# MuMuJun97/semantic_slam_mapping

Hardware: AMD Instinct MI355X
Metric: frames/sec semantic-mapping, 640x480 RGB-D (higher is better)
Workload: dtype u8; 1 GPU; configs[1]: synthetic 640x480 RGB-D + precomputed 12-class masks, 1k frames per GPU, ORB 1000 kp/frame, 5 ref frames, leaf 0.10 m; frames_per_gpu=1000, frames_all_gpus=1000, batch_frames=250, matcher_halo_frames=0, parallelism=single GPU

## Files before the change

### semantic_slam_mapping_amd/csrc/kernels_map.hip

```cpp
#include "ssm_internal.h"
#include <cstring>
#include <cmath>

#define MK_W 64
#define MK_H 16
__global__ void __launch_bounds__(256)
mask_kernel(const uint8_t* __restrict__ sem, int w, int h, int tiles_x, uint8_t* __restrict__ mask)
{
    __shared__ uint8_t m0[MK_H + 4][MK_W + 4];
    __shared__ uint8_t m1[MK_H + 4][MK_W];
    const int tx0 = (blockIdx.x % tiles_x) * MK_W, ty0 = (blockIdx.x / tiles_x) * MK_H;
    const uint8_t* s = sem + (size_t)blockIdx.y * w * h * 3;
    for (int i = threadIdx.x; i < (MK_H + 4) * (MK_W + 4); i += 256) {
        const int ly = i / (MK_W + 4), lx = i - ly * (MK_W + 4);
        const int gx = tx0 + lx - 2, gy = ty0 + ly - 2;
        uint8_t v = 0;
        if (gx >= 0 && gx < w && gy >= 0 && gy < h) {
            const uint8_t* p = s + ((size_t)gy * w + gx) * 3;
            const int b = p[0], g = p[1], r = p[2];
            v = ((b == 0 && g == 64 && r == 64) || (b == 192 && g == 128 && r == 0)) ? 255 : 0;
        }
        m0[ly][lx] = v;
    }
    __syncthreads();
    for (int i = threadIdx.x; i < (MK_H + 4) * MK_W; i += 256) {
        const int ly = i / MK_W, lx = i - ly * MK_W;
        const uint8_t* p = &m0[ly][lx];
        m1[ly][lx] = p[0] | p[1] | p[2] | p[3] | p[4];
    }
    __syncthreads();
    uint8_t* dst = mask + (size_t)blockIdx.y * w * h;
    const int lx = threadIdx.x & 63;
    for (int ly = threadIdx.x >> 6; ly < MK_H; ly += 4) {
        const int gx = tx0 + lx, gy = ty0 + ly;
        if (gx < w && gy < h) dst[(size_t)gy * w + gx] = m1[ly][lx] | m1[ly+1][lx] | m1[ly+2][lx] | m1[ly+3][lx] | m1[ly+4][lx];
    }
}
hipError_t k_moving_mask(const uint8_t* sem, int n, int w, int h, uint8_t* mask, hipStream_t s)
{
    const int tx = (w + MK_W - 1) / MK_W, ty = (h + MK_H - 1) / MK_H;
    mask_kernel<<<dim3(tx * ty, n), 256, 0, s>>>(sem, w, h, tx, mask);
    return hipGetLastError();
}

#define BP_PIX 1024
int backproject_chunks(int w, int h) { return (w * h + BP_PIX - 1) / BP_PIX; }

__device__ __forceinline__ bool bp_keep(int d, int mk, int b, int g, int r, double maxd)
{
    if (d == 0) return false;
    if ((double)d > maxd) return false;
    if (mk == 255) return false;
    if ((b == 128 && g == 128 && r == 128) || (b == 128 && g == 192 && r == 192) || (b == 192 && g == 128 && r == 0)) return false;
    return true;
}
__global__ void __launch_bounds__(256)
bp_count_kernel(const uint16_t* __restrict__ depth, const uint8_t* __restrict__ sem, const uint8_t* __restrict__ mask,
                int npix, double maxd, int chunks, int32_t* __restrict__ chunk_cnt)
{
    __shared__ int wsum[4];
    const size_t fo = (size_t)blockIdx.y * npix;
    const int p0 = blockIdx.x * BP_PIX + threadIdx.x * 4;
    int c = 0;
#pragma unroll
    for (int i = 0; i < 4; i++) {
        const int p = p0 + i;
        if (p < npix) {
            const uint8_t* s = sem + (fo + p) * 3;
            c += bp_keep(depth[fo + p], mask[fo + p], s[0], s[1], s[2], maxd);
        }
    }
#pragma unroll
    for (int o = 32; o > 0; o >>= 1) c += __shfl_xor(c, o, 64);
    if ((threadIdx.x & 63) == 0) wsum[threadIdx.x >> 6] = c;
    __syncthreads();
    if (threadIdx.x == 0) chunk_cnt[blockIdx.y * chunks + blockIdx.x] = wsum[0] + wsum[1] + wsum[2] + wsum[3];
}
__global__ void __launch_bounds__(1024)
bp_scan_kernel(const int32_t* __restrict__ chunk_cnt, int n, int chunks, int64_t* __restrict__ chunk_off,
               int32_t* __restrict__ npoints, int64_t* __restrict__ total)
{
    __shared__ long long part[1024];
    const int tot = n * chunks, tid = threadIdx.x;
    const int per = (tot + 1023) / 1024;
    const int b = tid * per, e = min(b + per, tot);
    long long s = 0;
    for (int i = b; i < e; i++) s += chunk_cnt[i];
    part[tid] = s;
    __syncthreads();
    for (int o = 1; o < 1024; o <<= 1) {
        long long v = tid >= o ? part[tid - o] : 0;
        __syncthreads();
        part[tid] += v;
        __syncthreads();
    }
    long long run = part[tid] - s;
    for (int i = b; i < e; i++) { chunk_off[i] = run; run += chunk_cnt[i]; }
    if (tid == 1023) *total = part[1023];
    __syncthreads();
    for (int f = tid; f < n; f += 1024) {
        int t = 0;
        for (int c = 0; c < chunks; c++) t += chunk_cnt[f * chunks + c];
        npoints[f] = t;
    }
}
__global__ void __launch_bounds__(256)
bp_emit_kernel(const uint16_t* __restrict__ depth, const uint8_t* __restrict__ rgb, const uint8_t* __restrict__ sem,
               const uint8_t* __restrict__ mask, const double* __restrict__ pose, int w, int npix, ssm_camera cam, double maxd,
               int chunks, const int64_t* __restrict__ chunk_off, ssm_point* __restrict__ out)
{
    __shared__ int wsum[4];
    const size_t fo = (size_t)blockIdx.y * npix;
    const int p0 = blockIdx.x * BP_PIX + threadIdx.x * 4;
    const int lane = threadIdx.x & 63, wv = threadIdx.x >> 6;
    bool k[4]; int c = 0;
#pragma unroll
    for (int i = 0; i < 4; i++) {
        const int p = p0 + i; k[i] = false;
        if (p < npix) {
            const uint8_t* s = sem + (fo + p) * 3;
            k[i] = bp_keep(depth[fo + p], mask[fo + p], s[0], s[1], s[2], maxd);
        }
        c += k[i];
    }
    int inc = c;
#pragma unroll
    for (int o = 1; o < 64; o <<= 1) { const int v = __shfl_up(inc, o, 64); if (lane >= o) inc += v; }
    if (lane == 63) wsum[wv] = inc;
    __syncthreads();
    int off = inc - c;
    for (int i = 0; i < wv; i++) off += wsum[i];
    if (c == 0) return;
    ssm_point* dst = out + chunk_off[blockIdx.y * chunks + blockIdx.x] + off;
    double T[12];
    const bool hasT = pose != nullptr;
    if (hasT) { const double* P = pose + (size_t)blockIdx.y * 16;
#pragma unroll
        for (int j = 0; j < 4; j++) { T[3*j] = P[4*j]; T[3*j+1] = P[4*j+1]; T[3*j+2] = P[4*j+2]; } }
#pragma unroll
    for (int i = 0; i < 4; i++) {
        if (!k[i]) continue;
        const int p = p0 + i;
        const int v = p / w, u = p - v * w;
        const int d = depth[fo + p];
        const float z = (float)((double)d / cam.scale);
        const float x = (float)(((double)u - cam.cx) * (double)z / cam.fx);
        const float y = (float)(((double)v - cam.cy) * (double)z / cam.fy);
        float ox = x, oy = y, oz = z;
        if (hasT) {
            const double X = x, Y = y, Z = z;
            ox = (float)(T[0] * X + T[3] * Y + T[6] * Z + T[9]);
            oy = (float)(T[1] * X + T[4] * Y + T[7] * Z + T[10]);
            oz = (float)(T[2] * X + T[5] * Y + T[8] * Z + T[11]);
        }
        const uint8_t* c3 = rgb + (fo + p) * 3;
        const uint8_t* s3 = sem + (fo + p) * 3;
        const int sb = s3[0], sg = s3[1], sr = s3[2];
        uint32_t label = 255;
        switch ((sb << 16) | (sg << 8) | sr) {
            case (128 << 16) | (128 << 8) | 128: label = 0; break;   case (0 << 16) | (0 << 8) | 128: label = 1; break;
            case (128 << 16) | (192 << 8) | 192: label = 2; break;   case (0 << 16) | (69 << 8) | 255: label = 3; break;
            case (128 << 16) | (64 << 8) | 128: label = 4; break;    case (222 << 16) | (40 << 8) | 60: label = 5; break;
            case (0 << 16) | (128 << 8) | 128: label = 6; break;     case (128 << 16) | (128 << 8) | 192: label = 7; break;
            case (128 << 16) | (64 << 8) | 64: label = 8; break;     case (128 << 16) | (0 << 8) | 64: label = 9; break;
            case (0 << 16) | (64 << 8) | 64: label = 10; break;      case (192 << 16) | (128 << 8) | 0: label = 11; break;
        }
        uint4 lo, hi;
        lo.x = __float_as_uint(ox); lo.y = __float_as_uint(oy); lo.z = __float_as_uint(oz); lo.w = __float_as_uint(1.0f);
        hi.x = (uint32_t)c3[0] | ((uint32_t)c3[1] << 8) | ((uint32_t)c3[2] << 16); hi.y = label; hi.z = 0; hi.w = 0;
        uint4* o = reinterpret_cast<uint4*>(dst);
        o[0] = lo; o[1] = hi;
        dst++;
    }
}
hipError_t k_backproject(const uint16_t* depth, const uint8_t* rgb, const uint8_t* sem, const uint8_t* mask,
                         const double* pose, int n, int w, int h, ssm_camera cam, double max_distance,
                         int32_t* chunk_cnt, int64_t* chunk_off, int32_t* npoints, int64_t* total,
                         ssm_point* out, hipStream_t s)
{
    const int npix = w * h, chunks = backproject_chunks(w, h);
    const double maxd = max_distance * cam.scale;
    bp_count_kernel<<<dim3(chunks, n), 256, 0, s>>>(depth, sem, mask, npix, maxd, chunks, chunk_cnt);
    bp_scan_kernel<<<1, 1024, 0, s>>>(chunk_cnt, n, chunks, chunk_off, npoints, total);
    bp_emit_kernel<<<dim3(chunks, n), 256, 0, s>>>(depth, rgb, sem, mask, pose, w, npix, cam, maxd, chunks, chunk_off, out);
    return hipGetLastError();
}

#define VOX_PROBE_LIMIT 128u
__device__ __forceinline__ uint32_t vox_hash(int64_t key)
{
    uint64_t z = (uint64_t)key * 0x9E3779B97F4A7C15ULL;
    z ^= z >> 29; z *= 0xBF58476D1CE4E5B9ULL; z ^= z >> 32;
    return (uint32_t)z;
}
__device__ __forceinline__ ssm_voxel* vox_find_or_insert(ssm_voxel* tab, int cap_log2, int64_t key, int32_t* counters, uint32_t* occ)
{
    const uint32_t mask = (1u << cap_log2) - 1u;
    const uint32_t limit = mask < VOX_PROBE_LIMIT - 1u ? mask : VOX_PROBE_LIMIT - 1u;
    uint32_t slot = vox_hash(key) & mask;
    for (uint32_t probe = 0; probe <= limit; probe++, slot = (slot + 1) & mask) {
        unsigned long long* kp = reinterpret_cast<unsigned long long*>(&tab[slot].key);
        unsigned long long cur = __hip_atomic_load(kp, __ATOMIC_RELAXED, __HIP_MEMORY_SCOPE_AGENT);
        if (cur == (unsigned long long)key) return &tab[slot];
        if (cur == (unsigned long long)SSM_VOX_EMPTY) {
            const unsigned long long prev = atomicCAS(kp, (unsigned long long)SSM_VOX_EMPTY, (unsigned long long)key);
            if (prev == (unsigned long long)SSM_VOX_EMPTY) { const int i = atomicAdd(&counters[0], 1); occ[i] = slot; return &tab[slot]; }
            if (prev == (unsigned long long)key) return &tab[slot];
        }
    }
    return nullptr;
}
typedef __attribute__((address_space(1))) ssm_voxel g_voxel;
__device__ __forceinline__ g_voxel* vox_overflow_slot(int32_t* counters)
{
    const int cap = counters[3];
    g_voxel* buf = (g_voxel*)*reinterpret_cast<ssm_voxel* const*>(counters + 4);
    const int i = cap > 0 ? atomicAdd(&counters[2], 1) : cap;
    if (i >= cap) { atomicOr(&counters[1], 1); return nullptr; }
    return buf + i;
}
__device__ __forceinline__ void vox_store_record(g_voxel* o, const ssm_voxel& sv)
{
    o->key = sv.key; o->sx = sv.sx; o->sy = sv.sy; o->sz = sv.sz; o->sr = sv.sr; o->sg = sv.sg; o->sb = sv.sb; o->n = sv.n;
    for (int c = 0; c < 12; c++) o->hist[c] = sv.hist[c];
}
__device__ __forceinline__ void vox_overflow_packed(int32_t* counters, long long key, long long sx, long long sy, long long sz, unsigned r, unsigned g, unsigned b, unsigned n, const unsigned* hist6)
{
    unsigned h[6];
    for (int c = 0; c < 6; c++) h[c] = hist6[c];
    g_voxel* o = vox_overflow_slot(counters);
    if (!o) return;
    o->key = key; o->sx = sx; o->sy = sy; o->sz = sz; o->sr = r; o->sg = g; o->sb = b; o->n = n;
    for (int c = 0; c < 12; c++) o->hist[c] = (h[c >> 1] >> (16 * (c & 1))) & 0xFFFF;
}
__device__ __forceinline__ void vox_overflow_one(int32_t* counters, long long key, long long sx, long long sy, long long sz, unsigned long long sr, unsigned long long sg,
                                              unsigned long long sb, unsigned long long n, uint32_t lab)
{
    g_voxel* o = vox_overflow_slot(counters);
    if (!o) return;
    o->key = key; o->sx = sx; o->sy = sy; o->sz = sz; o->sr = sr; o->sg = sg; o->sb = sb; o->n = n;
#pragma unroll
    for (int c = 0; c < 12; c++) o->hist[c] = (uint32_t)c == lab ? (uint32_t)n : 0u;
}
__device__ __forceinline__ void vox_add(ssm_voxel* v, long long sx, long long sy, long long sz, unsigned long long sr, unsigned long long sg,
                                        unsigned long long sb, unsigned long long n)
{
    atomicAdd(reinterpret_cast<unsigned long long*>(&v->sx), (unsigned long long)sx);
    atomicAdd(reinterpret_cast<unsigned long long*>(&v->sy), (unsigned long long)sy);
    atomicAdd(reinterpret_cast<unsigned long long*>(&v->sz), (unsigned long long)sz);
    atomicAdd(reinterpret_cast<unsigned long long*>(&v->sr), sr);
    atomicAdd(reinterpret_cast<unsigned long long*>(&v->sg), sg);
    atomicAdd(reinterpret_cast<unsigned long long*>(&v->sb), sb);
    atomicAdd(reinterpret_cast<unsigned long long*>(&v->n), n);
}
__global__ void vox_clear_kernel(ssm_voxel* __restrict__ tab, uint32_t* __restrict__ occ, int32_t* __restrict__ counters, int full, unsigned slots)
{
    const unsigned n = full ? slots : (unsigned)counters[0];
    for (unsigned i = blockIdx.x * blockDim.x + threadIdx.x; i < n; i += gridDim.x * blockDim.x) {
        ssm_voxel* v = &tab[full ? i : occ[i]];
        uint4* p = reinterpret_cast<uint4*>(v);
        const uint4 z = make_uint4(0, 0, 0, 0);
#pragma unroll
        for (int k = 1; k < 7; k++) p[k] = z;
        p[0] = make_uint4(0xFFFFFFFFu, 0xFFFFFFFFu, 0, 0);
    }
}
__global__ void vox_reset_counters(int32_t* counters) { counters[0] = 0; counters[1] = 0; counters[2] = 0; counters[6] = 0; counters[7] = 0; }
hipError_t k_voxel_clear(ssm_voxel* tab, int cap_log2, int32_t* counters, hipStream_t s)
{
    const int full = cap_log2 < 0; const unsigned slots = 1u << (full ? -cap_log2 : cap_log2);
    uint32_t* occ = reinterpret_cast<uint32_t*>(tab + slots);
    vox_clear_kernel<<<2048, 256, 0, s>>>(tab, occ, counters, full, slots);
    vox_reset_counters<<<1, 1, 0, s>>>(counters);
    return hipGetLastError();
}

__global__ void __launch_bounds__(256)
vox_insert_kernel(const ssm_point* __restrict__ pts, const int64_t* __restrict__ n_dev, int64_t n_max, float inv_leaf,
                  ssm_voxel* __restrict__ tab, int cap_log2, int32_t* __restrict__ counters)
{
    const int64_t n = n_dev ? min(*n_dev, n_max) : n_max;
    uint32_t* occ = reinterpret_cast<uint32_t*>(tab + (1u << cap_log2));
    const int lane = threadIdx.x & 63;
    const int64_t stride = (int64_t)gridDim.x * blockDim.x;
    for (int64_t base = (int64_t)blockIdx.x * blockDim.x; base < n; base += stride) {
        const int64_t i = base + threadIdx.x;
        const bool valid = i < n;
        long long key = -2, sx = 0, sy = 0, sz = 0; uint32_t rg = 0, bn = 0, label = 255;
        if (valid) {
            const uint4* p = reinterpret_cast<const uint4*>(pts + i);
            const uint4 lo = p[0], hi = p[1];
            const float x = __uint_as_float(lo.x), y = __uint_as_float(lo.y), z = __uint_as_float(lo.z);
            const float fi = floorf(x * inv_leaf), fj = floorf(y * inv_leaf), fk = floorf(z * inv_leaf);
            const long long vi = (long long)(int)fi + (1 << 20), vj = (long long)(int)fj + (1 << 20), vk = (long long)(int)fk + (1 << 20);
            key = (vk << 42) | (vj << 21) | vi;
            if (!(fabsf(fi) < 1048576.0f && fabsf(fj) < 1048576.0f && fabsf(fk) < 1048576.0f)) { key = -1; atomicOr(&counters[1], 2); }
            sx = __double2ll_rn((double)x * 16777216.0); sy = __double2ll_rn((double)y * 16777216.0); sz = __double2ll_rn((double)z * 16777216.0);
            rg = ((hi.x >> 16) & 255) | (((hi.x >> 8) & 255) << 16);
            bn = (hi.x & 255) | (1u << 16);
            label = hi.y;
        }
        const long long kprev = __shfl_up(key, 1, 64);
        const bool head = lane == 0 || kprev != key;
        const unsigned long long heads = __ballot(head);
        const int start = 63 - __clzll(heads & (~0ull >> (63 - lane)));
#pragma unroll
        for (int o = 1; o < 64; o <<= 1) {
            const long long ax = __shfl_up(sx, o, 64), ay = __shfl_up(sy, o, 64), az = __shfl_up(sz, o, 64);
            const uint32_t arg = __shfl_up(rg, o, 64), abn = __shfl_up(bn, o, 64);
            if (lane - o >= start) { sx += ax; sy += ay; sz += az; rg += arg; bn += abn; }
        }
        const bool tail = lane == 63 || ((heads >> (lane + 1)) & 1ull);
        unsigned long long lb[12];
#pragma unroll
        for (int c = 0; c < 12; c++) lb[c] = __ballot(label == (uint32_t)c);
        if (valid && tail && key >= 0) {
            ssm_voxel* v = vox_find_or_insert(tab, cap_log2, key, counters, occ);
            const unsigned long long run = (~0ull >> (63 - lane)) & (~0ull << start);
            if (v) {
                vox_add(v, sx, sy, sz, rg & 0xFFFF, rg >> 16, bn & 0xFFFF, bn >> 16);
#pragma unroll
                for (int c = 0; c < 12; c++) { const int k = __popcll(lb[c] & run); if (k) atomicAdd(&v->hist[c], (uint32_t)k); }
            } else if (g_voxel* o = vox_overflow_slot(counters)) {
                o->key = key; o->sx = sx; o->sy = sy; o->sz = sz; o->sr = rg & 0xFFFF; o->sg = rg >> 16; o->sb = bn & 0xFFFF; o->n = bn >> 16;
#pragma unroll
                for (int c = 0; c < 12; c++) o->hist[c] = (uint32_t)__popcll(lb[c] & run);
            }
        }
    }
}
hipError_t k_voxel_insert(const ssm_point* pts, const int64_t* n_dev, int64_t n_max, float leaf, ssm_voxel* tab,
                          int cap_log2, int32_t* counters, hipStream_t s)
{
    if (n_max <= 0) return hipSuccess;
    int64_t blocks = (n_max + 255) / 256; if (blocks > 8192) blocks = 8192;
    vox_insert_kernel<<<(int)blocks, 256, 0, s>>>(pts, n_dev, n_max, 1.0f / leaf, tab, cap_log2, counters);
    return hipGetLastError();
}
template <int CTRL, int ROW_MASK>
__device__ __forceinline__ int dpp_mov0(int v) { return __builtin_amdgcn_update_dpp(0, v, CTRL, ROW_MASK, 0xF, false); }
template <int CTRL, int ROW_MASK>
__device__ __forceinline__ long long dpp_mov0_ll(long long v)
{
    const int lo = dpp_mov0<CTRL, ROW_MASK>((int)(unsigned)(unsigned long long)v), hi = dpp_mov0<CTRL, ROW_MASK>((int)((unsigned long long)v >> 32));
    return (long long)(((unsigned long long)(unsigned)hi << 32) | (unsigned)lo);
}
struct RunAcc { long long sx, sy, sz; uint32_t r, g, b, n; };
__device__ __forceinline__ void run_scan(RunAcc& a, int lane, int start)
{
#define RS_STEP(CTRL, MASK, COND)                                                                                   \
    {   const long long tx = dpp_mov0_ll<CTRL, MASK>(a.sx), ty = dpp_mov0_ll<CTRL, MASK>(a.sy), tz = dpp_mov0_ll<CTRL, MASK>(a.sz); \
        const uint32_t t1 = (uint32_t)dpp_mov0<CTRL, MASK>((int)a.r), t2 = (uint32_t)dpp_mov0<CTRL, MASK>((int)a.g);             \
        const uint32_t t3 = (uint32_t)dpp_mov0<CTRL, MASK>((int)a.b), t4 = (uint32_t)dpp_mov0<CTRL, MASK>((int)a.n);             \
        if (COND) { a.sx += tx; a.sy += ty; a.sz += tz; a.r += t1; a.g += t2; a.b += t3; a.n += t4; } }
    const int li = lane & 15, row = lane >> 4;
    RS_STEP(0x111, 0xF, (li >= 1 && lane - 1 >= start))
    RS_STEP(0x112, 0xF, (li >= 2 && lane - 2 >= start))
    RS_STEP(0x114, 0xF, (li >= 4 && lane - 4 >= start))
    RS_STEP(0x118, 0xF, (li >= 8 && lane - 8 >= start))
    RS_STEP(0x142, 0xA, ((row & 1) && start < 16 * row))
    RS_STEP(0x143, 0xC, (row >= 2 && start < 32))
#undef RS_STEP
}
__device__ __forceinline__ long long f64_to_ll_rn(double v)
{
    const double M = 6755399441055744.0;
    return __double_as_longlong(v + M) - __double_as_longlong(M);
}
__device__ __forceinline__ uint32_t label_hash_entry(int k)
{
    switch (k) {
        case 10: return (0u << 24) | 128u | (128u << 8) | (128u << 16);   case 1:  return (1u << 24) | 0u | (0u << 8) | (128u << 16);
        case 2:  return (2u << 24) | 128u | (192u << 8) | (192u << 16);   case 9:  return (3u << 24) | 0u | (69u << 8) | (255u << 16);
        case 4:  return (4u << 24) | 128u | (64u << 8) | (128u << 16);    case 13: return (5u << 24) | 222u | (40u << 8) | (60u << 16);
        case 14: return (6u << 24) | 0u | (128u << 8) | (128u << 16);     case 11: return (7u << 24) | 128u | (128u << 8) | (192u << 16);
        case 3:  return (8u << 24) | 128u | (64u << 8) | (64u << 16);     case 12: return (9u << 24) | 128u | (0u << 8) | (64u << 16);
        case 7:  return (10u << 24) | 0u | (64u << 8) | (64u << 16);      case 15: return (11u << 24) | 192u | (128u << 8) | (0u << 16);
    }
    return 0xFF000001u;
}
#define MS_SLOTS 256
#ifndef MS_MINB
#define MS_MINB 4
#endif
#define MS_CH 3
struct LdsVox { long long key, sx, sy, sz; unsigned r, g, b, n; unsigned hist[6]; };
__device__ __forceinline__ uint32_t label_of_bgr24(uint32_t bgr)
{
    switch (bgr) {
        case 128u | (128u << 8) | (128u << 16): return 0;   case 0u | (0u << 8) | (128u << 16): return 1;
        case 128u | (192u << 8) | (192u << 16): return 2;   case 0u | (69u << 8) | (255u << 16): return 3;
        case 128u | (64u << 8) | (128u << 16): return 4;    case 222u | (40u << 8) | (60u << 16): return 5;
        case 0u | (128u << 8) | (128u << 16): return 6;     case 128u | (128u << 8) | (192u << 16): return 7;
        case 128u | (64u << 8) | (64u << 16): return 8;     case 128u | (0u << 8) | (64u << 16): return 9;
        case 0u | (64u << 8) | (64u << 16): return 10;      case 192u | (128u << 8) | (0u << 16): return 11;
    }
    return 255;
}
__device__ __forceinline__ void vox_direct(long long key, uint32_t lab, long long sx, long long sy, long long sz, unsigned r, unsigned g, unsigned b, unsigned n,
                ssm_voxel* tab, int cap_log2, int32_t* counters, uint32_t* occ)
{
    ssm_voxel* v = vox_find_or_insert(tab, cap_log2, key, counters, occ);
    if (__builtin_expect(v != nullptr, 1)) { vox_add(v, sx, sy, sz, r, g, b, n); if (lab < 12) atomicAdd(&v->hist[lab], n); }
    else vox_overflow_one(counters, key, sx, sy, sz, r, g, b, n, lab);
}
__device__ __forceinline__ void lds_vox_update(LdsVox* lt, long long key, uint32_t lab, const RunAcc& f,
                                               ssm_voxel* tab, int cap_log2, int32_t* counters, uint32_t* occ)
{
    uint32_t slot = vox_hash(key) & (MS_SLOTS - 1);
    LdsVox* e = nullptr;
    for (int probe = 0; probe < MS_SLOTS; probe++, slot = (slot + 1) & (MS_SLOTS - 1)) {
        const unsigned long long prev = atomicCAS(reinterpret_cast<unsigned long long*>(&lt[slot].key), (unsigned long long)SSM_VOX_EMPTY, (unsigned long long)key);
        if (prev == (unsigned long long)SSM_VOX_EMPTY || prev == (unsigned long long)key) { e = &lt[slot]; break; }
    }
    if (__builtin_expect(e != nullptr, 1)) {
        atomicAdd(reinterpret_cast<unsigned long long*>(&e->sx), (unsigned long long)f.sx);
        atomicAdd(reinterpret_cast<unsigned long long*>(&e->sy), (unsigned long long)f.sy);
        atomicAdd(reinterpret_cast<unsigned long long*>(&e->sz), (unsigned long long)f.sz);
        atomicAdd(&e->r, f.r); atomicAdd(&e->g, f.g); atomicAdd(&e->b, f.b); atomicAdd(&e->n, f.n);
        if (lab < 12) atomicAdd(&e->hist[lab >> 1], f.n << (16 * (lab & 1)));
    } else vox_direct(key, lab, f.sx, f.sy, f.sz, f.r, f.g, f.b, f.n, tab, cap_log2, counters, occ);
}
__device__ __forceinline__ void wave_flush(LdsVox* lt, long long key, uint32_t lab, RunAcc f, int lane,
                                           ssm_voxel* tab, int cap_log2, int32_t* counters, uint32_t* occ)
{
    const long long kprev = dpp_mov0_ll<0x138, 0xF>(key);
    const uint32_t lprev = (uint32_t)dpp_mov0<0x138, 0xF>((int)lab);
    const bool head = lane == 0 || kprev != key || lprev != lab;
    const unsigned long long heads = __ballot(head);
    const int start = 63 - __clzll(heads & (~0ull >> (63 - lane)));
    run_scan(f, lane, start);
    const bool tail = lane == 63 || ((heads >> (lane + 1)) & 1ull);
    if (key >= 0 && tail) lds_vox_update(lt, key, lab, f, tab, cap_log2, counters, occ);
}
__device__ __forceinline__ double markstein_div(double n, double f, double r)
{
    double q = n * r;
    q = fma(fma(-q, f, n), r, q);
    return fma(fma(-q, f, n), r, q);
}
#define MS2_MINB 4
#define MS2_SKIP_CAP 65536
#define MS2_CB_WORDS (MS_CH * 256 + 6 * 256)
template <bool FASTDIV, bool REDO>
__global__ void __launch_bounds__(256, MS2_MINB)
map_stream2_kernel(const uint16_t* __restrict__ depth, const uint8_t* __restrict__ rgb, const uint8_t* __restrict__ sem,
                   const double* __restrict__ pose, int w, int h, ssm_camera cam, MapDiv md, double maxd,
                   float inv_leaf, ssm_voxel* __restrict__ tab, int cap_log2, int32_t* __restrict__ counters, int32_t* __restrict__ npoints, uint32_t mul_wpr,
                   int32_t* __restrict__ skip, int hw, int tag, int gx)
{
    __shared__ LdsVox lt[MS_SLOTS];
    __shared__ int s_npts, s_skip;
    int bx_ = blockIdx.x, by_ = blockIdx.y;
    if (REDO) { const int id = skip[blockIdx.x] & 0xFFFFFF; by_ = id / gx; bx_ = id - by_ * gx; }
    const int bx = bx_, by = by_;
    if (!REDO && threadIdx.x == 0) {
        int sk = 0;
        if (__hip_atomic_load(&counters[2], __ATOMIC_RELAXED, __HIP_MEMORY_SCOPE_AGENT) > hw) {
            const int i = atomicAdd(&counters[6], 1);
            if (i < MS2_SKIP_CAP) skip[i] = (tag << 24) | (by * gx + bx); else atomicOr(&counters[1], 1);
            sk = 1;
        }
        s_skip = sk;
    }
    __shared__ uint16_t vlist[4][1024];
    __shared__ uint16_t cbits[MS2_CB_WORDS];
    const int tid = threadIdx.x, lane = tid & 63, wv = tid >> 6;
    const int wpr = w >> 4, words = wpr * h;
    const int bw0 = bx * MS_CH * 256;
    const int ry0 = (int)__umulhi((uint32_t)bw0, mul_wpr) - 2;
    const int own0 = bw0 - ry0 * wpr, own1 = min(bw0 + MS_CH * 256, words) - ry0 * wpr;
    const uint32_t tab_entry = label_hash_entry(lane & 15);
    uint32_t labs[MS_CH][2];
#pragma unroll
    for (int ch = 0; ch < MS_CH; ch++) {
        labs[ch][0] = labs[ch][1] = 0u;
        const int wi = (bx * MS_CH + ch) * 256 + wv * 64 + lane;
        const bool inw = wi < words;
        if ((bx * MS_CH + ch) * 256 + wv * 64 < words) {
            const uint4* ps = reinterpret_cast<const uint4*>(sem + ((size_t)by * words + (inw ? wi : words - 1)) * 48);
            const uint4 S0 = ps[0], S1 = ps[1], S2 = ps[2];
            const uint32_t ss[13] = {S0.x, S0.y, S0.z, S0.w, S1.x, S1.y, S1.z, S1.w, S2.x, S2.y, S2.z, S2.w, 0u};
            uint32_t bits = 0;
#pragma unroll
            for (int k = 0; k < 16; k++) {
                const int o = 3 * k;
                const uint32_t sbgr = ((o & 3) ? __builtin_amdgcn_alignbyte(ss[(o >> 2) + 1], ss[o >> 2], o & 3) : ss[o >> 2]) & 0xFFFFFFu;
                const uint32_t ent = (uint32_t)__shfl((int)tab_entry, (int)((sbgr * 0x7589a82bu) >> 28), 64);
                const uint32_t lab = (ent & 0xFFFFFFu) == sbgr ? ent >> 24 : 15u;
                labs[ch][k >> 3] |= lab << (4 * (k & 7));
                bits |= (uint32_t)(lab == 10u || lab == 11u) << k;
            }
            if (inw) cbits[wi - ry0 * wpr] = (uint16_t)bits;
        }
    }
    {
        const int ry1 = (int)__umulhi((uint32_t)(min(bw0 + MS_CH * 256, words) - 1), mul_wpr) + 2;
        const int ncw = (ry1 - ry0 + 1) * wpr, nhalo = ncw - (own1 - own0);
        for (int j = tid; j < nhalo; j += 256) {
            const int i = j < own0 ? j : j + (own1 - own0);
            const int rr = (int)__umulhi((uint32_t)i, mul_wpr), gy = ry0 + rr;
            uint32_t bits = 0;
            if (gy >= 0 && gy < h) {
                const uint4* p = reinterpret_cast<const uint4*>(sem + ((size_t)by * words + (size_t)((long long)ry0 * wpr + i)) * 48);
                const uint4 a = p[0], b = p[1], c = p[2];
                const uint32_t d[13] = {a.x, a.y, a.z, a.w, b.x, b.y, b.z, b.w, c.x, c.y, c.z, c.w, 0u};
#pragma unroll
                for (int k = 0; k < 16; k++) {
                    const int o = 3 * k;
                    const uint32_t bgr = ((o & 3) ? __builtin_amdgcn_alignbyte(d[(o >> 2) + 1], d[o >> 2], o & 3) : d[o >> 2]) & 0xFFFFFFu;
                    bits |= (uint32_t)(bgr == (0u | (64u << 8) | (64u << 16)) || bgr == (192u | (128u << 8) | (0u << 16))) << k;
                }
            }
            cbits[i] = (uint16_t)bits;
        }
    }
    for (int i = tid; i < MS_SLOTS; i += 256) {
        lt[i].key = SSM_VOX_EMPTY; lt[i].sx = 0; lt[i].sy = 0; lt[i].sz = 0; lt[i].r = lt[i].g = lt[i].b = lt[i].n = 0;
#pragma unroll
        for (int k = 0; k < 6; k++) lt[i].hist[k] = 0;
    }
    if (tid == 0) s_npts = 0;
    __syncthreads();
    if (!REDO && s_skip) return;
    uint32_t* occ = reinterpret_cast<uint32_t*>(tab + (1u << cap_log2));
    int kept = 0; bool out_of_range = false;
    double T[12];
    const bool hasT = pose != nullptr;
    if (hasT) { const double* P = pose + (size_t)by * 16;
#pragma unroll
        for (int j = 0; j < 4; j++) { T[3*j] = P[4*j]; T[3*j+1] = P[4*j+1]; T[3*j+2] = P[4*j+2]; } }
    const int dmax = maxd >= 65535.0 ? 65535 : (int)maxd;
#pragma unroll 1
    for (int ch = 0; ch < MS_CH; ch++) {
    const int wbase = (bx * MS_CH + ch) * 256 + wv * 64;
    const int wi = wbase + lane;
    uint32_t keepbits = 0;
    uint32_t lab4[2] = {labs[0][0], labs[0][1]};
#pragma unroll
    for (int c_ = 1; c_ < MS_CH; c_++) { lab4[0] = ch == c_ ? labs[c_][0] : lab4[0]; lab4[1] = ch == c_ ? labs[c_][1] : lab4[1]; }
    if (wi < words) {
        const size_t gw = (size_t)by * words + wi;
        const int gy = (int)__umulhi((uint32_t)wi, mul_wpr), xw = wi - gy * wpr;
        const uint4* pd = reinterpret_cast<const uint4*>(depth + gw * 16);
        const uint4 D0 = pd[0], D1 = pd[1];
        const uint16_t* cb = cbits + (gy - ry0 - 2) * wpr + xw;
        uint32_t vl = 0, vc = 0, vr = 0;
#pragma unroll
        for (int r5 = 0; r5 < 5; r5++) { vc |= cb[r5 * wpr]; if (xw > 0) vl |= cb[r5 * wpr - 1]; if (xw + 1 < wpr) vr |= cb[r5 * wpr + 1]; }
        const unsigned long long win = (unsigned long long)vl | ((unsigned long long)vc << 16) | ((unsigned long long)vr << 32);
        const uint32_t moving = (uint32_t)((win >> 14) | (win >> 15) | (win >> 16) | (win >> 17) | (win >> 18)) & 0xFFFFu;
        const uint32_t dd[8] = {D0.x, D0.y, D0.z, D0.w, D1.x, D1.y, D1.z, D1.w};
#pragma unroll
        for (int k = 0; k < 16; k++) {
            const int d = (dd[k >> 1] >> (16 * (k & 1))) & 0xFFFF;
            const uint32_t lab = (lab4[k >> 3] >> (4 * (k & 7))) & 15u;
            const bool gated = (0x805u >> lab) & 1u;
            keepbits |= (uint32_t)(d != 0 && d <= dmax && !gated) << k;
        }
        keepbits &= ~moving;
    }
    const uint32_t cnt = __popc(keepbits);
    uint32_t incl = cnt;
    incl += (uint32_t)__builtin_amdgcn_update_dpp(0, (int)incl, 0x111, 0xF, 0xF, false);
    incl += (uint32_t)__builtin_amdgcn_update_dpp(0, (int)incl, 0x112, 0xF, 0xF, false);
    incl += (uint32_t)__builtin_amdgcn_update_dpp(0, (int)incl, 0x114, 0xF, 0xF, false);
    incl += (uint32_t)__builtin_amdgcn_update_dpp(0, (int)incl, 0x118, 0xF, 0xF, false);
    incl += (uint32_t)__builtin_amdgcn_update_dpp(0, (int)incl, 0x142, 0xA, 0xF, false);
    incl += (uint32_t)__builtin_amdgcn_update_dpp(0, (int)incl, 0x143, 0xC, 0xF, false);
    const int V = __builtin_amdgcn_readlane((int)incl, 63);
    kept += (int)cnt;
    {
        int base = (int)(incl - cnt);
#pragma unroll
        for (int k = 0; k < 16; k++)
            if ((keepbits >> k) & 1u) vlist[wv][base++] = (uint16_t)((lane << 4) | k | (((lab4[k >> 3] >> (4 * (k & 7))) & 15u) << 10));
    }
    const int P = (V + 63) >> 6;
    long long k0 = -2, k1 = -2; uint32_t l0 = 255, l1 = 255; RunAcc a0, a1;
    a0.sx = a0.sy = a0.sz = 0; a0.r = a0.g = a0.b = a0.n = 0; a1 = a0;
    __builtin_amdgcn_wave_barrier();
    struct PixIn { uint32_t ent; int d; uint32_t c01, c2; };
    auto fetch = [&](int e, PixIn& q) {
        q.ent = vlist[wv][min(e, V - 1)];
        const int sl = (q.ent >> 4) & 63, k = q.ent & 15;
        const size_t gp = ((size_t)by * words + wbase + sl) * 16 + k;
        q.d = depth[gp];
        uint16_t c01; __builtin_memcpy(&c01, rgb + gp * 3, 2);
        q.c01 = c01; q.c2 = rgb[gp * 3 + 2];
    };
    auto pixel = [&](int e, const PixIn& q, long long& key, uint32_t& lab, RunAcc& p) {
        const uint32_t ent = q.ent;
        const int sl = (ent >> 4) & 63, k = ent & 15;
        lab = (ent >> 10) == 15u ? 255u : (ent >> 10);
        const int d = q.d;
        const uint32_t cbgr = q.c01 | (q.c2 << 16);
        const int wip = wbase + sl;
        const int gy = (int)__umulhi((uint32_t)wip, mul_wpr), gx = ((wip - gy * wpr) << 4) + k;
        const double yf = (double)gy - cam.cy;
        float x, y, z;
        if (FASTDIV) {
            z = (float)markstein_div((double)d, cam.scale, md.rscale);
            x = (float)markstein_div(((double)gx - cam.cx) * (double)z, cam.fx, md.rfx);
            y = (float)markstein_div(yf * (double)z, cam.fy, md.rfy);
        } else {
            z = (float)((double)d / cam.scale);
            x = (float)(((double)gx - cam.cx) * (double)z / cam.fx);
            y = (float)(yf * (double)z / cam.fy);
        }
        float ox = x, oy = y, oz = z;
        if (hasT) {
            const double X = x, Y = y, Z = z;
            ox = (float)(T[0] * X + T[3] * Y + T[6] * Z + T[9]);
            oy = (float)(T[1] * X + T[4] * Y + T[7] * Z + T[10]);
            oz = (float)(T[2] * X + T[5] * Y + T[8] * Z + T[11]);
        }
        const float fi = floorf(ox * inv_leaf), fj = floorf(oy * inv_leaf), fk = floorf(oz * inv_leaf);
        const long long vi = (long long)(int)fi + (1 << 20), vj = (long long)(int)fj + (1 << 20), vk = (long long)(int)fk + (1 << 20);
        key = (vk << 42) | (vj << 21) | vi;
        if (!(fabsf(fi) < 1048576.0f && fabsf(fj) < 1048576.0f && fabsf(fk) < 1048576.0f)) { key = -1; if (e < V) out_of_range = true; }
        p.sx = f64_to_ll_rn((double)ox * 16777216.0); p.sy = f64_to_ll_rn((double)oy * 16777216.0); p.sz = f64_to_ll_rn((double)oz * 16777216.0);
        p.b = cbgr & 255; p.g = (cbgr >> 8) & 255; p.r = cbgr >> 16; p.n = 1;
    };
    auto accumulate = [&](long long key, uint32_t lab, const RunAcc& p) {
        if (k1 == -2 && (k0 == -2 || (k0 == key && l0 == lab))) {
            k0 = key; l0 = lab; a0.sx += p.sx; a0.sy += p.sy; a0.sz += p.sz; a0.r += p.r; a0.g += p.g; a0.b += p.b; a0.n += 1;
        } else if (k1 == -2 || (k1 == key && l1 == lab)) {
            k1 = key; l1 = lab; a1.sx += p.sx; a1.sy += p.sy; a1.sz += p.sz; a1.r += p.r; a1.g += p.g; a1.b += p.b; a1.n += 1;
        } else {
            if (k1 >= 0) lds_vox_update(lt, k1, l1, a1, tab, cap_log2, counters, occ);
            k1 = key; l1 = lab; a1 = p;
        }
    };
    constexpr int MS2_UN = 2;
    PixIn cur[MS2_UN], nxt[MS2_UN];
    if (P > 0) {
#pragma unroll
        for (int u = 0; u < MS2_UN; u++) fetch(lane * P + u, nxt[u]);
    }
#pragma unroll 1
    for (int i = 0; i < P; i += MS2_UN) {
        long long kk[MS2_UN]; uint32_t ll[MS2_UN]; RunAcc pp[MS2_UN];
#pragma unroll
        for (int u = 0; u < MS2_UN; u++) { cur[u] = nxt[u]; fetch(lane * P + i + MS2_UN + u, nxt[u]); }
#pragma unroll
        for (int u = 0; u < MS2_UN; u++) pixel(lane * P + i + u, cur[u], kk[u], ll[u], pp[u]);
#pragma unroll
        for (int u = 0; u < MS2_UN; u++) if (i + u < P && lane * P + i + u < V) accumulate(kk[u], ll[u], pp[u]);
    }
    if (k0 >= 0) lds_vox_update(lt, k0, l0, a0, tab, cap_log2, counters, occ);
    if (k1 >= 0) lds_vox_update(lt, k1, l1, a1, tab, cap_log2, counters, occ);
    __builtin_amdgcn_wave_barrier();
    }
#pragma unroll
    for (int o = 32; o > 0; o >>= 1) kept += __shfl_xor(kept, o, 64);
    if (lane == 0 && kept) atomicAdd(&s_npts, kept);
    if (__ballot(out_of_range) && lane == 0) atomicOr(&counters[1], 2);
    __syncthreads();
    for (int i = tid; i < MS_SLOTS; i += 256) {
        if (lt[i].key == SSM_VOX_EMPTY) continue;
        ssm_voxel* v = vox_find_or_insert(tab, cap_log2, lt[i].key, counters, occ);
        if (__builtin_expect(!v, 0)) { vox_overflow_packed(counters, lt[i].key, lt[i].sx, lt[i].sy, lt[i].sz, lt[i].r, lt[i].g, lt[i].b, lt[i].n, lt[i].hist); continue; }
        vox_add(v, lt[i].sx, lt[i].sy, lt[i].sz, lt[i].r, lt[i].g, lt[i].b, lt[i].n);
#pragma unroll
        for (int c = 0; c < 12; c++) { const uint32_t k = (lt[i].hist[c >> 1] >> (16 * (c & 1))) & 0xFFFF; if (k) atomicAdd(&v->hist[c], k); }
    }
    if (tid == 0 && s_npts) atomicAdd(&npoints[by], s_npts);
}
bool k_map_div(const ssm_camera& cam, MapDiv& md)
{
    md.rscale = 1.0 / cam.scale; md.rfx = 1.0 / cam.fx; md.rfy = 1.0 / cam.fy;
    auto plain = [](double f) {
        uint64_t b; memcpy(&b, &f, 8);
        const uint64_t man = b & 0xFFFFFFFFFFFFFull; const int ex = (int)((b >> 52) & 0x7FF);
        return f > 0 && ex > 0 && ex < 0x7FF && man != 0xFFFFFFFFFFFFFull;
    };
    bool ok = plain(cam.scale) && plain(cam.fx) && plain(cam.fy);
    for (int d = 0; d < 65536 && ok; d++) {
        double q = (double)d * md.rscale; q = std::fma(std::fma(-q, cam.scale, (double)d), md.rscale, q); q = std::fma(std::fma(-q, cam.scale, (double)d), md.rscale, q);
        if (q != (double)d / cam.scale) ok = false;
    }
    return ok;
}
int k_map_fuse_blocks_per_frame(int w, int h) { const int words = (w >> 4) * h; return (words + 256 * MS_CH - 1) / (256 * MS_CH); }
int k_map_fuse_block_records(void) { return MS_CH * 4096; }
int k_map_fuse_resident_blocks(void) { return 256 * MS2_MINB; }
int k_map_fuse_skip_cap(void) { return MS2_SKIP_CAP; }
hipError_t k_map_fuse(const uint16_t* depth, const uint8_t* rgb, const uint8_t* sem, const double* pose, int n, int w, int h,
                      ssm_camera cam, const MapDiv& md, bool fast, double max_distance, float leaf,
                      ssm_voxel* tab, int cap_log2, int32_t* counters, int32_t* npoints, hipStream_t s, int32_t* skip, int hw, int tag, const int32_t* redo_ids, int nredo)
{
    const int wpr = w >> 4, words = wpr * h;
    if (!((long long)words * wpr < (1ll << 32) && wpr <= 256)) return hipErrorInvalidValue;
    if (nredo <= 0) { const hipError_t e = hipMemsetAsync(npoints, 0, sizeof(int32_t) * n, s); if (e != hipSuccess) return e; }
    const int gx = (words + 256 * MS_CH - 1) / (256 * MS_CH);
    const dim3 grid(gx, n);
    const uint32_t mul_wpr = (uint32_t)(((1ull << 32) + wpr - 1) / wpr);
    const double maxd = max_distance * cam.scale; const float il = 1.0f / leaf;
    if (nredo > 0) {
        int32_t* ids = const_cast<int32_t*>(redo_ids);
        if (fast) map_stream2_kernel<true, true><<<nredo, 256, 0, s>>>(depth, rgb, sem, pose, w, h, cam, md, maxd, il, tab, cap_log2, counters, npoints, mul_wpr, ids, 0, tag, gx);
        else map_stream2_kernel<false, true><<<nredo, 256, 0, s>>>(depth, rgb, sem, pose, w, h, cam, md, maxd, il, tab, cap_log2, counters, npoints, mul_wpr, ids, 0, tag, gx);
    } else {
        if (fast) map_stream2_kernel<true, false><<<grid, 256, 0, s>>>(depth, rgb, sem, pose, w, h, cam, md, maxd, il, tab, cap_log2, counters, npoints, mul_wpr, skip, hw, tag, gx);
        else map_stream2_kernel<false, false><<<grid, 256, 0, s>>>(depth, rgb, sem, pose, w, h, cam, md, maxd, il, tab, cap_log2, counters, npoints, mul_wpr, skip, hw, tag, gx);
    }
    return hipGetLastError();
}

__global__ void vox_merge_kernel(const ssm_voxel* __restrict__ src, int n, ssm_voxel* __restrict__ tab, int cap_log2, int32_t* __restrict__ counters)
{
    uint32_t* occ = reinterpret_cast<uint32_t*>(tab + (1u << cap_log2));
    const int i = blockIdx.x * blockDim.x + threadIdx.x;
    if (i >= n) return;
    const ssm_voxel sv = src[i];
    ssm_voxel* v = vox_find_or_insert(tab, cap_log2, sv.key, counters, occ);
    if (!v) { if (g_voxel* o = vox_overflow_slot(counters)) vox_store_record(o, sv); return; }
    vox_add(v, sv.sx, sv.sy, sv.sz, sv.sr, sv.sg, sv.sb, sv.n);
    for (int c = 0; c < 12; c++) if (sv.hist[c]) atomicAdd(&v->hist[c], sv.hist[c]);
}
__global__ void vox_rehash_kernel(const ssm_voxel* __restrict__ src, const uint32_t* __restrict__ src_occ, const int32_t* __restrict__ src_counters,
                                  ssm_voxel* __restrict__ tab, int cap_log2, int32_t* __restrict__ counters)
{
    uint32_t* occ = reinterpret_cast<uint32_t*>(tab + (1u << cap_log2));
    const int n = src_counters[0];
    for (int i = blockIdx.x * blockDim.x + threadIdx.x; i < n; i += gridDim.x * blockDim.x) {
        const ssm_voxel sv = src[src_occ[i]];
        ssm_voxel* v = vox_find_or_insert(tab, cap_log2, sv.key, counters, occ);
        if (!v) { if (g_voxel* o = vox_overflow_slot(counters)) vox_store_record(o, sv); continue; }
        vox_add(v, sv.sx, sv.sy, sv.sz, sv.sr, sv.sg, sv.sb, sv.n);
        for (int c = 0; c < 12; c++) if (sv.hist[c]) atomicAdd(&v->hist[c], sv.hist[c]);
    }
}
hipError_t k_voxel_rehash(const ssm_voxel* src, int src_cap_log2, ssm_voxel* tab, int cap_log2, int32_t* counters, hipStream_t s)
{
    const uint32_t* socc = reinterpret_cast<const uint32_t*>(src + ((size_t)1 << src_cap_log2));
    const int32_t* scnt = reinterpret_cast<const int32_t*>(socc + ((size_t)1 << src_cap_log2));
    vox_rehash_kernel<<<1024, 256, 0, s>>>(src, socc, scnt, tab, cap_log2, counters);
    return hipGetLastError();
}
hipError_t k_voxel_merge(const ssm_voxel* src, int n, ssm_voxel* tab, int cap_log2, int32_t* counters, hipStream_t s)
{
    if (n <= 0) return hipSuccess;
    vox_merge_kernel<<<(n + 255) / 256, 256, 0, s>>>(src, n, tab, cap_log2, counters);
    return hipGetLastError();
}
__global__ void vox_compact_kernel(const ssm_voxel* __restrict__ tab, const uint32_t* __restrict__ occ, const int32_t* __restrict__ counters,
                                   ssm_voxel* __restrict__ out, int32_t* __restrict__ n_out)
{
    const int n = counters[0];
    if (blockIdx.x == 0 && threadIdx.x == 0) *n_out = n;
    for (int i = blockIdx.x * blockDim.x + threadIdx.x; i < n; i += gridDim.x * blockDim.x) {
        const uint4* s = reinterpret_cast<const uint4*>(&tab[occ[i]]);
        uint4* d = reinterpret_cast<uint4*>(&out[i]);
#pragma unroll
        for (int k = 0; k < 7; k++) d[k] = s[k];
    }
}
hipError_t k_voxel_compact(const ssm_voxel* tab, int cap_log2, ssm_voxel* out, int32_t* n_out, hipStream_t s)
{
    const uint32_t* occ = reinterpret_cast<const uint32_t*>(tab + (1u << cap_log2));
    const int32_t* counters = reinterpret_cast<const int32_t*>(occ + (1u << cap_log2));
    vox_compact_kernel<<<1024, 256, 0, s>>>(tab, occ, counters, out, n_out);
    return hipGetLastError();
}
__global__ void vox_gather_points_kernel(const ssm_voxel* __restrict__ c, const uint32_t* __restrict__ order, int n, ssm_point* __restrict__ out)
{
    const int i = blockIdx.x * blockDim.x + threadIdx.x;
    if (i >= n) return;
    const ssm_voxel v = c[order[i]];
    const double nn = (double)v.n;
    const float x = (float)(((double)v.sx / nn) * (1.0 / 16777216.0));
    const float y = (float)(((double)v.sy / nn) * (1.0 / 16777216.0));
    const float z = (float)(((double)v.sz / nn) * (1.0 / 16777216.0));
    const uint32_t r = (uint32_t)(v.sr / v.n), g = (uint32_t)(v.sg / v.n), b = (uint32_t)(v.sb / v.n);
    uint32_t best = 0, lab = 255;
#pragma unroll
    for (int k = 0; k < 12; k++) if (v.hist[k] > best) { best = v.hist[k]; lab = k; }
    uint4 lo, hi;
    lo.x = __float_as_uint(x); lo.y = __float_as_uint(y); lo.z = __float_as_uint(z); lo.w = __float_as_uint(1.0f);
    hi.x = b | (g << 8) | (r << 16); hi.y = lab; hi.z = 0; hi.w = 0;
    uint4* o = reinterpret_cast<uint4*>(out + i);
    o[0] = lo; o[1] = hi;
}
hipError_t k_voxel_gather_points(const ssm_voxel* compact, const uint32_t* order, int n, ssm_point* out, hipStream_t s)
{
    if (n <= 0) return hipSuccess;
    vox_gather_points_kernel<<<(n + 255) / 256, 256, 0, s>>>(compact, order, n, out);
    return hipGetLastError();
}
__global__ void vox_gather_table_kernel(const ssm_voxel* __restrict__ c, const uint32_t* __restrict__ order, int n, ssm_voxel* __restrict__ out)
{
    const int i = blockIdx.x * blockDim.x + threadIdx.x;
    if (i >= n) return;
    const uint4* s = reinterpret_cast<const uint4*>(&c[order[i]]);
    uint4* d = reinterpret_cast<uint4*>(&out[i]);
#pragma unroll
    for (int k = 0; k < 7; k++) d[k] = s[k];
}
hipError_t k_voxel_gather_table(const ssm_voxel* compact, const uint32_t* order, int n, ssm_voxel* out, hipStream_t s)
{
    if (n <= 0) return hipSuccess;
    vox_gather_table_kernel<<<(n + 255) / 256, 256, 0, s>>>(compact, order, n, out);
    return hipGetLastError();
}
__device__ __forceinline__ int f2ord(float f) { int i = __float_as_int(f); return i >= 0 ? i : i ^ 0x7FFFFFFF; }
__global__ void vox_bounds_kernel(const ssm_point* __restrict__ pts, int n, int* __restrict__ mm)
{
    int mn[3] = {0x7FFFFFFF, 0x7FFFFFFF, 0x7FFFFFFF}, mx[3] = {(int)0x80000000, (int)0x80000000, (int)0x80000000};
    for (int i = blockIdx.x * blockDim.x + threadIdx.x; i < n; i += gridDim.x * blockDim.x) {
        const float4 p = *reinterpret_cast<const float4*>(pts + i);
        const int a[3] = {f2ord(p.x), f2ord(p.y), f2ord(p.z)};
#pragma unroll
        for (int k = 0; k < 3; k++) { mn[k] = min(mn[k], a[k]); mx[k] = max(mx[k], a[k]); }
    }
#pragma unroll
    for (int k = 0; k < 3; k++) {
#pragma unroll
        for (int o = 32; o > 0; o >>= 1) { mn[k] = min(mn[k], __shfl_xor(mn[k], o, 64)); mx[k] = max(mx[k], __shfl_xor(mx[k], o, 64)); }
    }
    if ((threadIdx.x & 63) == 0) for (int k = 0; k < 3; k++) { atomicMin(&mm[k], mn[k]); atomicMax(&mm[3 + k], mx[k]); }
}
__global__ void vox_bounds_init(int* mm) { mm[0] = mm[1] = mm[2] = 0x7FFFFFFF; mm[3] = mm[4] = mm[5] = (int)0x80000000; }
hipError_t k_voxel_bounds(const ssm_point* pts, int n, float* minmax6, hipStream_t s)
{
    vox_bounds_init<<<1, 1, 0, s>>>(reinterpret_cast<int*>(minmax6));
    if (n > 0) vox_bounds_kernel<<<min((n + 255) / 256, 1024), 256, 0, s>>>(pts, n, reinterpret_cast<int*>(minmax6));
    return hipGetLastError();
}

struct PoseArg { double t[12]; };
__global__ void __launch_bounds__(256)
cloud_transform_kernel(const ssm_point* __restrict__ src, int n, PoseArg P, ssm_point* __restrict__ dst)
{
    const int i = blockIdx.x * blockDim.x + threadIdx.x;
    if (i >= n) return;
    ssm_point p = src[i];
    const double x = p.x, y = p.y, z = p.z;
    p.x = (float)(P.t[0] * x + P.t[3] * y + P.t[6] * z + P.t[9]);
    p.y = (float)(P.t[1] * x + P.t[4] * y + P.t[7] * z + P.t[10]);
    p.z = (float)(P.t[2] * x + P.t[5] * y + P.t[8] * z + P.t[11]);
    dst[i] = p;
}
hipError_t k_cloud_transform(const ssm_point* src, int n, const double* T, ssm_point* dst, hipStream_t s)
{
    if (n <= 0) return hipSuccess;
    if (!T) return hipMemcpyAsync(dst, src, (size_t)n * sizeof(ssm_point), hipMemcpyDeviceToDevice, s);
    PoseArg P;
    for (int c = 0; c < 4; c++) for (int r = 0; r < 3; r++) P.t[3 * c + r] = T[4 * c + r];
    cloud_transform_kernel<<<(n + 255) / 256, 256, 0, s>>>(src, n, P, dst);
    return hipGetLastError();
}
```

Before: 186,200 frames/s.

## Carry leftover compacted pixels across chunks so waves process full 64-lane batches

Each wave's compacted pixel list is now processed only in multiples of 64 entries per chunk. The remainder is carried to the front of the list for the next chunk, and an extra final iteration drains what is left. List entries encode the source chunk in two extra bits, and the odd trailing trip is peeled out of the unrolled loop. This aims to cut idle lanes and per-entry bounds checks in the pixel/accumulate loop, at the cost of one more loop pass, an LDS shuffle of the carry, and a slightly larger LDS list.

```diff
diff --git a/semantic_slam_mapping_amd/csrc/kernels_map.hip b/semantic_slam_mapping_amd/csrc/kernels_map.hip
--- a/semantic_slam_mapping_amd/csrc/kernels_map.hip
+++ b/semantic_slam_mapping_amd/csrc/kernels_map.hip
@@ -441,6 +441,8 @@
 }
 #define MS2_MINB 4
 #define MS2_SKIP_CAP 65536
+#define MS2_VL 1088
+static_assert(MS_CH <= 4, "a list entry has two bits for the chunk it comes from: widen the entry before raising MS_CH");
 #define MS2_CB_WORDS (MS_CH * 256 + 6 * 256)
 template <bool FASTDIV, bool REDO>
 __global__ void __launch_bounds__(256, MS2_MINB)
@@ -463,9 +465,9 @@
         }
         s_skip = sk;
     }
-    __shared__ uint16_t vlist[4][1024];
+    __shared__ uint16_t vlist[4][MS2_VL];
     __shared__ uint16_t cbits[MS2_CB_WORDS];
-    const int tid = threadIdx.x, lane = tid & 63, wv = tid >> 6;
+    const int tid = threadIdx.x, lane = tid & 63, wv = __builtin_amdgcn_readfirstlane(tid >> 6);
     const int wpr = w >> 4, words = wpr * h;
     const int bw0 = bx * MS_CH * 256;
     const int ry0 = (int)__umulhi((uint32_t)bw0, mul_wpr) - 2;
@@ -531,15 +533,17 @@
 #pragma unroll
         for (int j = 0; j < 4; j++) { T[3*j] = P[4*j]; T[3*j+1] = P[4*j+1]; T[3*j+2] = P[4*j+2]; } }
     const int dmax = maxd >= 65535.0 ? 65535 : (int)maxd;
+    const int wb0 = bw0 + wv * 64;
+    int carry = 0;
 #pragma unroll 1
-    for (int ch = 0; ch < MS_CH; ch++) {
-    const int wbase = (bx * MS_CH + ch) * 256 + wv * 64;
-    const int wi = wbase + lane;
+    for (int ch = 0; ch <= MS_CH; ch++) {
+    const bool last = ch == MS_CH;
+    const int wi = wb0 + ch * 256 + lane;
     uint32_t keepbits = 0;
     uint32_t lab4[2] = {labs[0][0], labs[0][1]};
 #pragma unroll
     for (int c_ = 1; c_ < MS_CH; c_++) { lab4[0] = ch == c_ ? labs[c_][0] : lab4[0]; lab4[1] = ch == c_ ? labs[c_][1] : lab4[1]; }
-    if (wi < words) {
+    if (!last && wi < words) {
         const size_t gw = (size_t)by * words + wi;
         const int gy = (int)__umulhi((uint32_t)wi, mul_wpr), xw = wi - gy * wpr;
         const uint4* pd = reinterpret_cast<const uint4*>(depth + gw * 16);
@@ -571,31 +575,34 @@
     const int V = __builtin_amdgcn_readlane((int)incl, 63);
     kept += (int)cnt;
     {
-        int base = (int)(incl - cnt);
+        int base = carry + (int)(incl - cnt);
+        const uint32_t hi = (uint32_t)(lane << 4) | ((uint32_t)ch << 14);
 #pragma unroll
         for (int k = 0; k < 16; k++)
-            if ((keepbits >> k) & 1u) vlist[wv][base++] = (uint16_t)((lane << 4) | k | (((lab4[k >> 3] >> (4 * (k & 7))) & 15u) << 10));
-    }
-    const int P = (V + 63) >> 6;
+            if ((keepbits >> k) & 1u) vlist[wv][base++] = (uint16_t)(hi | k | (((lab4[k >> 3] >> (4 * (k & 7))) & 15u) << 10));
+    }
+    const int total = carry + V;
+    const int Q = last ? (total + 63) >> 6 : total >> 6;
     long long k0 = -2, k1 = -2; uint32_t l0 = 255, l1 = 255; RunAcc a0, a1;
     a0.sx = a0.sy = a0.sz = 0; a0.r = a0.g = a0.b = a0.n = 0; a1 = a0;
     __builtin_amdgcn_wave_barrier();
     struct PixIn { uint32_t ent; int d; uint32_t c01, c2; };
     auto fetch = [&](int e, PixIn& q) {
-        q.ent = vlist[wv][min(e, V - 1)];
+        q.ent = vlist[wv][min(e, total - 1)];
         const int sl = (q.ent >> 4) & 63, k = q.ent & 15;
-        const size_t gp = ((size_t)by * words + wbase + sl) * 16 + k;
+        const size_t gp = ((size_t)by * words + wb0 + ((q.ent >> 14) << 8) + sl) * 16 + k;
         q.d = depth[gp];
         uint16_t c01; __builtin_memcpy(&c01, rgb + gp * 3, 2);
         q.c01 = c01; q.c2 = rgb[gp * 3 + 2];
     };
-    auto pixel = [&](int e, const PixIn& q, long long& key, uint32_t& lab, RunAcc& p) {
+    auto pixel = [&](bool real, const PixIn& q, long long& key, uint32_t& lab, RunAcc& p) {
         const uint32_t ent = q.ent;
         const int sl = (ent >> 4) & 63, k = ent & 15;
-        lab = (ent >> 10) == 15u ? 255u : (ent >> 10);
+        const uint32_t lb4 = (ent >> 10) & 15u;
+        lab = lb4 == 15u ? 255u : lb4;
         const int d = q.d;
         const uint32_t cbgr = q.c01 | (q.c2 << 16);
-        const int wip = wbase + sl;
+        const int wip = wb0 + (int)((ent >> 14) << 8) + sl;
         const int gy = (int)__umulhi((uint32_t)wip, mul_wpr), gx = ((wip - gy * wpr) << 4) + k;
         const double yf = (double)gy - cam.cy;
         float x, y, z;
@@ -618,7 +625,7 @@
         const float fi = floorf(ox * inv_leaf), fj = floorf(oy * inv_leaf), fk = floorf(oz * inv_leaf);
         const long long vi = (long long)(int)fi + (1 << 20), vj = (long long)(int)fj + (1 << 20), vk = (long long)(int)fk + (1 << 20);
         key = (vk << 42) | (vj << 21) | vi;
-        if (!(fabsf(fi) < 1048576.0f && fabsf(fj) < 1048576.0f && fabsf(fk) < 1048576.0f)) { key = -1; if (e < V) out_of_range = true; }
+        if (!(fabsf(fi) < 1048576.0f && fabsf(fj) < 1048576.0f && fabsf(fk) < 1048576.0f)) { key = -1; if (real) out_of_range = true; }
         p.sx = f64_to_ll_rn((double)ox * 16777216.0); p.sy = f64_to_ll_rn((double)oy * 16777216.0); p.sz = f64_to_ll_rn((double)oz * 16777216.0);
         p.b = cbgr & 255; p.g = (cbgr >> 8) & 255; p.r = cbgr >> 16; p.n = 1;
     };
@@ -634,22 +641,38 @@
     };
     constexpr int MS2_UN = 2;
     PixIn cur[MS2_UN], nxt[MS2_UN];
-    if (P > 0) {
-#pragma unroll
-        for (int u = 0; u < MS2_UN; u++) fetch(lane * P + u, nxt[u]);
-    }
+    if (Q > 0) {
+#pragma unroll
+        for (int u = 0; u < MS2_UN; u++) fetch(lane * Q + u, nxt[u]);
+    }
+    const int Qe = Q & ~(MS2_UN - 1);
 #pragma unroll 1
-    for (int i = 0; i < P; i += MS2_UN) {
+    for (int i = 0; i < Qe; i += MS2_UN) {
         long long kk[MS2_UN]; uint32_t ll[MS2_UN]; RunAcc pp[MS2_UN];
 #pragma unroll
-        for (int u = 0; u < MS2_UN; u++) { cur[u] = nxt[u]; fetch(lane * P + i + MS2_UN + u, nxt[u]); }
-#pragma unroll
-        for (int u = 0; u < MS2_UN; u++) pixel(lane * P + i + u, cur[u], kk[u], ll[u], pp[u]);
-#pragma unroll
-        for (int u = 0; u < MS2_UN; u++) if (i + u < P && lane * P + i + u < V) accumulate(kk[u], ll[u], pp[u]);
+        for (int u = 0; u < MS2_UN; u++) { cur[u] = nxt[u]; fetch(lane * Q + i + MS2_UN + u, nxt[u]); }
+#pragma unroll
+        for (int u = 0; u < MS2_UN; u++) pixel(true, cur[u], kk[u], ll[u], pp[u]);
+#pragma unroll
+        for (int u = 0; u < MS2_UN; u++) accumulate(kk[u], ll[u], pp[u]);
+    }
+    if (Q & 1) {
+        static_assert(MS2_UN == 2, "the peeled trip takes the one entry that is left of a pair");
+        long long kk; uint32_t ll; RunAcc pp;
+        const bool real = lane * Q + Qe < total;
+        pixel(real, nxt[0], kk, ll, pp);
+        if (real) accumulate(kk, ll, pp);
     }
     if (k0 >= 0) lds_vox_update(lt, k0, l0, a0, tab, cap_log2, counters, occ);
     if (k1 >= 0) lds_vox_update(lt, k1, l1, a1, tab, cap_log2, counters, occ);
+    carry = total - (Q << 6);
+    __builtin_amdgcn_wave_barrier();
+    if (!last && Q > 0 && carry > 0) {
+        uint16_t t = 0;
+        if (lane < carry) t = vlist[wv][(Q << 6) + lane];
+        __builtin_amdgcn_wave_barrier();
+        if (lane < carry) vlist[wv][lane] = t;
+    }
     __builtin_amdgcn_wave_barrier();
     }
 #pragma unroll
```

Result: no change. 188,200 frames/s (median of 6 runs) (+1.0%).
